# casselineau/Tracer

Hardware: AMD Instinct MI355X
Metric: Mray-bounces/s on Sandia NSTTF field (higher is better)
Workload: dtype f64

## Files before the change

tracer_amd/csrc/trc_device.h:

```cpp
#ifndef TRC_DEVICE_H
#define TRC_DEVICE_H

#include <hip/hip_runtime.h>
#include "trc_core.h"
#include "trc_bounds.h"
#include "trc_footprint.h"
#include "trc_forms.h"

struct FluxMapDev {
    int32_t surf, nu, nv, chart;
    int64_t edges_u, edges_v;
    int64_t bins;
    double proj[12];
};
static_assert(sizeof(FluxMapDev) == 136, "tests/shade_cases.py (SIZEOF_FLUXMAPDEV) restates this size in the sums of the LDS images");

struct DScene {
    const double *recs;
    const double *opt;
    const int32_t *sflags;
    const double *extra;
    int32_t stride, n_surf, n_extra, has_kd;
    const int32_t *kd_a, *kd_b, *kd_leaf, *kd_always;
    const double *kd_split;
// ... 321 lines not shown

#ifndef TALLY_PARTS
#define TALLY_PARTS 16
#endif

#define CN(k) ((k) << 4)
#define CN_WORDS (32 << 4)
enum StreamCounter {
    CW_Q1 = 0,
    CW_Q3 = 1,
    CW_HIT_LIST = 2,
    CW_ACT_OUT = 3,
    CW_OVERFLOW = 4,
    CW_ACT_IN = 5,
    CW_HITS = 6,
    CW_ALIVE = 7,
    CW_SLOTS = 8,
    CW_GEN_LIST = 9,
    CW_FP_LIST = 10,
    CW_TERM_LIST = 11,
    CW_TERM_HITS = 12,
    CW_CLS_HITS = 13,
    CW_STATS = 16,
    CW_CLS_LIST = 24
};
enum StreamOverflow : unsigned long long {
    CW_OVF_RETRY = 1,
    CW_OVF_FAIL = 2
};

struct StreamWs {
    long long cap;
    long long room;
    long long q3_cap;
    long long act_room;
    SRayGeo *geo;
    SRayAux *aux;
    uint32_t *q1_slot;
    float4 *q1_a, *q1_b;
    uint32_t *q3_slot, *q3_surf;
    SCand *q3n;
    uint32_t *hit_slot;
    uint32_t *hit_surf;
    double *hit_t;
    uint32_t *gen_list;
    uint32_t *fq_ray, *fq_cell;
    uint32_t *act[2];
// ... 32 lines not shown
    FpDev fp;
    int static_first;
    int lds_recs;
    int lds_tables;
    int lds_fm_bins;
    int lds_extra;
    int bounce_no;
    int bg_occ_words;
    int split_terminal;
    unsigned chunk_thit;
    int search;
    int shade_cls;
    int shade_term_cls;
    long long act_base0;
    unsigned chunk_hitbuf;
    const uint32_t *hl_slot, *hl_surf;
    const double *hl_t;
    long long hl_room;
    int hl_cn;
    unsigned part_chunk[3];
    int part_static[3];
    CarryIn carry;
    const float *clear_tab;
};

template <class ARGS>
__device__ __forceinline__ const ARGS *kernel_args_again() {
    static_assert(std::is_trivially_copyable<ARGS>::value, "the block is read as the bytes the launch copied into the segment");
    auto p = __builtin_amdgcn_kernarg_segment_ptr();
    asm volatile("" : "+s"(p));
    return (const ARGS *)p;
}

#define TRC_SURF_CLS_SHIFT 17
#define TRC_SURF_CLS_MASK 0x3
template <int THREADS>
__device__ __forceinline__ int wg_next(int i) {
    if constexpr (THREADS > 0) return i + THREADS;
    else return i + blockDim.x;
}

__device__ __forceinline__ void nearest_linked(const SCand *q3n, uint32_t k, double &t, int &s) {
    while (k != SQ_INVALID) {
        const SCand c = q3n[k];
        if (c.t < t || (c.t == t && (int)c.surf < s)) { t = c.t; s = (int)c.surf; }
        k = c.next;
// ... 255 lines not shown
```

tracer_amd/csrc/trc_forms.h:

```cpp
#ifndef TRC_FORMS_H
#define TRC_FORMS_H

#include <cstdio>
#include "trc_bounds.h"
#include "trc_footprint.h"

#define SC_THREADS 512
#define SC_GEN_CAP 1024
#define SF_THREADS(FLAT) ((FLAT) ? 1024 : 768)
#define SF2_DERIVES_CELL(FLAT, LDS) ((FLAT) || (LDS))
#ifndef SW_LEAFCAP
#define SW_LEAFCAP 16
#endif
#ifndef SW_LIST_T
#define SW_LIST_T uint16_t
#endif
#ifndef SW_THREADS
#define SW_THREADS 256
#endif
#define SB_THREADS 1024
#define SB_THREADS_OF(GRIDM) (SB_THREADS)
#define SA_THREADS 1024
#ifndef SHC_THREADS
#define SHC_THREADS 1024
// ... 77 lines not shown
    p.flags = flags;
    if (grid_cells) { p.grid_cells = grid_cells; p.grid_list = grid_list; }
    p.coop_waves = coop_waves;
    return p;
}
static inline size_t lds_need(const trc_lds_layout &L) { return L.end + L.slack; }
static inline size_t lds_request(const trc_lds_layout &L) { return lds_need(L) + 16; }
static inline size_t shade_lds_need(const trc_shade_parts &p) { const trc_shade_layout L = trc_shade_lds_layout(p); return L.end + L.slack; }

struct StreamKnobs {
    int search;
    bool fresh;
    bool bounce;
    bool first;
    bool coop;
    int absorb;
    bool static_chunks;
    bool room_set; long long room;
    long long q3_entries;
    int fp_cells;
    bool umask;
    int slots;
    bool clear = true;
};

struct trc_scene_facts {
    int n_surf, stride;
    bool accel_ok, accel_kd_ok, has_kd;
    int kd_nodes, kd_nleaf, kd_nalways, kd_depth;
    bool grid_ok, big_ok;
    int grid_cells, grid_list;
    int brute_list, n_unbounded;
    int big_occ_words;
    int n_fm_edges, fms_bytes, n_extra;
    long long fm_bins;
    bool chart;
    bool transfer;
    bool splits;
    bool walked;
    bool all_flat;
    bool simple;
    unsigned cls_moving, cls_all;
    bool any_term;
};
struct trc_call_facts {
    long long n;
    int flags;
    int src_kind;
    bool spec;
    bool carry;
    bool mat_dev;
    bool term_ok;
    int poly_src;
    int poly_walls;
};
struct trc_fp_facts {
    bool use;
    long long n_list;
    int M, Mc;
    bool has_generic;
    double cdf_end, coverage, ucoverage;
    int umask_words, Mu, Mv;
};
struct trc_facts { trc_scene_facts scene; trc_call_facts call; trc_fp_facts fp; StreamKnobs knobs; };

static inline void trc_scene_facts_fill(const trc_surface_desc *surfs, int n_surf, const trc_accel_host &A, bool walk, trc_scene_facts *s) {
    s->n_surf = n_surf;
    s->kd_depth = A.kd_depth;
    s->grid_ok = A.grid_ok; s->big_ok = A.big_ok;
    s->grid_cells = A.grid_off.empty() ? 0 : (int)A.grid_off.size() - 1;
    s->grid_list = (int)A.grid_list.size();
    s->brute_list = (int)A.brute_leaf.size();
    s->n_unbounded = (int)A.unbounded.size();
    s->big_occ_words = (int)A.big_occ.size();
    s->walked = walk;
    if (!walk) return;
    s->all_flat = s->simple = true;
    s->cls_moving = s->cls_all = 0u;
    s->any_term = false;
    for (int i = 0; i < n_surf; ++i) {
        const trc_surface_desc &sd = surfs[i];
        const bool flat = trc_gm_is_flat(sd.gm_kind);
        s->all_flat = s->all_flat && flat;
        s->simple = s->simple && flat && ((TRC_OPT_SIMPLE_MASK >> sd.optics_kind) & 1u);
        const unsigned bit = 1u << trc_shade_class_of(sd);
        s->cls_all |= bit;
        if (surface_ends_every_ray(sd)) s->any_term = true;
        else s->cls_moving |= bit;
    }
}

enum trc_kernel_family {
    TRC_K_NONE,
    TRC_K_CULL, TRC_K_UCULL,
    TRC_K_FRESH, TRC_K_FRESH2,
    TRC_K_BOUNCE,
    TRC_K_BOUNCE_COOP,
// ... 134 lines not shown
    return lds;
}

struct trc_stream_forms {
    int src_kind;
    int gridm;
    bool small_scene;
    trc_stage gen0, gen, walk, exact;
    trc_shade_stage shk[TRC_CLS_COUNT];
    int n_shk;
    bool multi;
    trc_stage cull, fresh, fresh_one;
    trc_stage cull_u;
    int cull_lu, cull_lv;
    double ulisted_share;
    trc_stage bounce, first, absorb;
    bool coop;
    bool use_fp, use_fused, use_first, use_absorb, absorb_inline;
    size_t lds_inline;
    double general_share;
    double listed_share;
    int search, lds_recs, lds_tally, lds_tables, lds_extra, lds_fm_bins, bg_occ_words, shade_term_cls, split_terminal;
    int poly_cells;
};

static inline trc_lds_parts trc_fresh_parts(const trc_facts &f, bool buie, bool lds, int queue_waves) {
    trc_fp_params P = {};
    P.Mc = f.fp.Mc;
    return fresh_lds_parts(f.scene.n_surf, f.scene.stride, P, f.fp.n_list, buie, lds, queue_waves);
}

static inline void trc_stream_form_general(trc_stream_forms &F, const trc_facts &f, const StreamPlan &plan) {
    const size_t b_recs = (size_t)f.scene.n_surf * f.scene.stride * 8;
    const size_t lds_exact = b_recs <= TRC_EXACT_RECS_LIMIT ? b_recs : 0;
    F.lds_recs = lds_exact ? 1 : 0;
    const int k = F.src_kind;
    const trc_kernel_id gen0 = trc_src_kind_is_lamp(k) ? trc_kid(TRC_K_GEN_LAMP, k)
                             : k == TRC_SRC_EMIT_THERMAL ? trc_kid(TRC_K_GEN_EMIT)
                             : (k == TRC_SRC_BUIE_DISK || k == TRC_SRC_PILLBOX_DISK || k == TRC_SRC_PILLBOX_RECT) ? trc_kid(TRC_K_GEN_SRC, k)
                             : trc_kid(TRC_K_GEN, 1, (k == TRC_SRC_BUIE_RECT || trc_src_kind_is_sunshape(k)) ? k : -1);
    F.gen0 = {gen0, 256, 0};
    F.gen = {trc_kid(TRC_K_GEN, 0, -1), 256, 0};
    F.walk = {trc_kid(TRC_K_WALK, SW_THREADS, plan.mode == 2), SW_THREADS, plan.lds_walk};
    F.exact = {trc_kid(TRC_K_EXACT), 256, lds_exact};
}

// ... 97 lines not shown
    F.bounce = {coop ? trc_kid(TRC_K_BOUNCE_COOP, 0, all_flat, 0) : trc_kid(TRC_K_BOUNCE, gridm, in_lds, 0, all_flat, 0), SB_THREADS_OF(gridm), request(false)};
    F.first = {coop ? trc_kid(TRC_K_BOUNCE_COOP, 1, all_flat, sun) : trc_kid(TRC_K_BOUNCE, gridm, in_lds, 1, 0, sun), SB_THREADS_OF(gridm), request(true)};
}

static inline void trc_stream_form_absorb(trc_stream_forms &F, const trc_facts &f) {
    const trc_scene_facts &sc = f.scene;
    if (!(F.use_fused && F.lds_tally && F.lds_tables && !f.call.carry)) return;
    auto need = [&](int img) { return shade_lds_need(trc_shade_lds_parts(img, true, sc.n_surf, sc.stride, sc.n_fm_edges, sc.fms_bytes, sc.n_extra, F.lds_fm_bins)); };
    const size_t lds_absorb = need(TRC_IMG_ABSORB);
    const bool fm_ok = sc.fm_bins == 0 || F.lds_fm_bins > 0;
    F.use_absorb = sc.any_term && fm_ok && !sc.chart && lds_absorb <= trc_shade_lds_limit(TRC_IMG_ABSORB, true) && !sc.transfer && f.call.term_ok && f.knobs.absorb != 0;
    if (!F.use_absorb) return;
    F.absorb = {trc_kid(TRC_K_ABSORB), SA_THREADS, lds_absorb};
    F.split_terminal = 1;
    const size_t extra_lds = need(TRC_IMG_INLINE);
    if (f.knobs.absorb != 1 && !(F.gridm == 2 && F.coop) && F.bounce.lds + extra_lds <= trc_shade_lds_limit(TRC_IMG_INLINE, true)) {
        F.absorb_inline = true;
        F.lds_inline = extra_lds;
        F.bounce.lds += extra_lds;
        F.split_terminal = 2;
    }
}

static inline bool trc_stream_decide(const trc_facts &f, const StreamPlan &plan, trc_stream_forms *out) {
    trc_stream_forms &F = *out;
    memset(&F, 0, sizeof(F));
    const int S = f.scene.n_surf;
    F.src_kind = f.call.src_kind;
    F.gridm = plan.mode == 2 ? 1 : (plan.mode == 3 ? 2 : 0);
    F.small_scene = S <= STREAM_SMALL_SURFACES && plan.mode != 1 && plan.walk_ok;
    if (F.small_scene && S <= STREAM_TINY_SURFACES) F.gridm = 3;
    F.search = plan.walk_ok ? plan.mode : 2;
    trc_stream_form_general(F, f, plan);
    if (!trc_stream_form_shade(F, f)) return false;
    trc_stream_form_fresh(F, f);
    trc_stream_form_bounce(F, f, plan);
    trc_stream_form_absorb(F, f);
    return true;
}

struct MegaPlan {
    bool m32;
    int threads;
    size_t lds;
    int lds_tally, lds_scene;
    trc_kernel_id id;
};
static inline MegaPlan mega_plan(const trc_scene_facts &sc, const trc_call_facts &c) {
    const int S = sc.n_surf;
    const bool accel = sc.has_kd && (c.flags & TRC_TRACE_ACCEL);
    const size_t b_buie = c.src_kind >= 0 ? (size_t)TRC_BUIE_STAGED * 8 : 0;
    const size_t b_tally = (size_t)(3 * S + 2) * 8;
    MegaPlan M = {false, 256, 0, 0, 0, {}};
    if (sc.accel_ok && S <= TRC_MAX_SURFACES16 && (!accel || (sc.accel_kd_ok && sc.kd_nodes <= COOP_MAX_NODES && sc.kd_depth <= COOP_MAX_DEPTH))) {
        const size_t b_acc = (size_t)6 * S * 4 + (accel ? ((size_t)2 * sc.kd_nodes * 4 + (size_t)sc.kd_nalways * 4 + (size_t)sc.kd_nleaf * 2)
                                                        : (8 + (size_t)sc.brute_list * 2)) +
                             (size_t)sc.n_unbounded * 4 + 32;
        const size_t b_wave = COOP_WAVE_BYTES(accel ? (sc.kd_depth > 0 ? sc.kd_depth : 1) : 1);
        for (int threads = 512; threads >= 256 && !M.m32; threads /= 2) {
            const size_t lds = b_buie + b_tally + b_acc + (size_t)(threads / 64) * b_wave;
// ... 42 lines not shown
```

tracer_amd/csrc/trc_shade.hip:

```cpp
#include "trc_device.h"

template <int CLS, bool FLATN, bool LDS, bool SPEC = false, bool CHART = false>
__global__ __launch_bounds__(SHC_THREADS) void k_s_shade_c(StreamParams S) {
    extern __shared__ double lds[];
    const FastParams &P = S.P;
    const DScene &sc = P.sc;
    const StreamWs &W = S.W;
    const int Sn = sc.n_surf;
    if (W.cnt[CN(CW_OVERFLOW)]) return;
    constexpr unsigned KINDS = CLS == TRC_CLS_MIRROR ? TRC_CLS_MIRROR_KINDS : TRC_CLS_DIFFUSE_KINDS;
    DScene L = sc;
    L.tally = W.tally_part + (size_t)(blockIdx.x % TALLY_PARTS) * (size_t)W.tally_n;
    double *l_tally = lds;
    double *cur = lds + (LDS ? 3 * Sn + 2 : 2);
    for (int i = threadIdx.x; i < (LDS ? 3 * Sn + 2 : 2); i += blockDim.x) l_tally[i] = 0.0;
    if (LDS) {
        double *l_recs = cur; cur += Sn * sc.stride;
        for (int i = threadIdx.x; i < Sn * sc.stride; i += blockDim.x) l_recs[i] = sc.recs[i];
        double *l_opt = cur; cur += 8 * Sn;
        for (int i = threadIdx.x; i < 8 * Sn; i += blockDim.x) l_opt[i] = sc.opt[i];
        double *l_edges = cur; cur += sc.n_fm_edges;
        for (int i = threadIdx.x; i < sc.n_fm_edges; i += blockDim.x) l_edges[i] = sc.fm_edges[i];
        FluxMapDev *l_fms = (FluxMapDev *)cur; cur += (sc.n_fm * sizeof(FluxMapDev) + 7) / 8;
        for (int i = threadIdx.x; i < sc.n_fm; i += blockDim.x) l_fms[i] = sc.fms[i];
// ... 3 lines not shown
        L.recs = l_recs; L.opt = l_opt; L.fm_edges = l_edges; L.fms = l_fms; L.fm_of_surf = l_fm_of; L.sflags = l_flags;
        cur = (double *)(((uintptr_t)(l_flags + Sn) + 7) & ~(uintptr_t)7);
        if (CLS != TRC_CLS_MIRROR) {
            double *l_extra = cur; cur += sc.n_extra;
            for (int i = threadIdx.x; i < sc.n_extra; i += blockDim.x) l_extra[i] = sc.extra[i];
            L.extra = l_extra;
        }
    }
    double *l_fm = nullptr;
    if (S.lds_fm_bins > 0) {
        l_fm = cur; cur += S.lds_fm_bins;
        for (int i = threadIdx.x; i < S.lds_fm_bins; i += blockDim.x) l_fm[i] = 0.0;
    }
    const double src_energy = P.src ? P.src->energy : 0.0;
    __syncthreads();
    long long nh = (long long)W.cnt[S.hl_cn];
    if (nh > S.hl_room) nh = S.hl_room;
    const long long padded = (nh + 63) & ~63ll;
    const unsigned wave_g = (blockIdx.x * blockDim.x + threadIdx.x) >> 6;
    WaveChunk ca = S.static_first ? chunk_init_static_at(S.chunk_act, (unsigned long long)S.act_base0 + (unsigned long long)wave_g * S.chunk_act) : chunk_init(S.chunk_act);
    WaveChunk hc = chunk_init(S.chunk_hitbuf);
    if (P.capture && wave_g < SHADE_MAX_WAVES) hit_chunk_resume(hc, W.hit_state + 2 * wave_g, S.hit_epoch);
    unsigned n_hit = 0, n_alive = 0;
    const int bounce0 = S.bounce_no;
    const bool aux_in = !P.src || bounce0 > 0;
    const long long stride = (long long)gridDim.x * blockDim.x;
    for (long long i = (long long)blockIdx.x * blockDim.x + threadIdx.x; i < padded; i += stride) {
        uint32_t slot = SQ_INVALID, hs = SQ_INVALID;
        double t = TRC_INF;
        SRayGeo g;
        g.px = g.py = g.pz = g.dx = g.dy = 0.0; g.dz = 1.0; g.head = SQ_INVALID; g.idx = 0u; g.tail = 0ull;
        bool have = false;
        if (i < nh) { slot = S.hl_slot[i]; hs = S.hl_surf[i]; t = S.hl_t[i]; }
        bool mine = false;
        int s = 0, fl = 0;
        if (slot != SQ_INVALID) {
            if (hs == SQ_INVALID) {
                g = W.geo[slot];
                have = true;
                t = TRC_INF;
                s = 0x7FFFFFFF;
                nearest_linked(W.q3n, g.head, t, s);
            } else s = (int)hs;
            if ((unsigned)s < (unsigned)Sn) {
                fl = L.sflags[s];
                const int cls = (fl >> TRC_SURF_CLS_SHIFT) & TRC_SURF_CLS_MASK;
                mine = (S.shade_term_cls >= 0 && (fl & TRC_SURF_TERMINAL)) ? (S.shade_term_cls == CLS) : (cls == CLS);
            }
            if (mine && !have) g = W.geo[slot];
        }
        const unsigned long long my_lanes = __ballot(mine);
        if (!my_lanes) continue;
        bool alive = false;
        int ts = -1;
        double tea = 0.0, tei = 0.0;
// ... 14 lines not shown
                }
                trc_normal(rec, hx, hy, hz, g.dx, g.dy, g.dz, &nx, &ny, &nz);
                trc_ray_out out[2];
                const unsigned long long rid = P.rid ? P.rid[S.base + (long long)g.idx] : (P.ray_offset + (unsigned long long)(S.base + (long long)g.idx));
                trc_shade_k<KINDS, false>(trc_rec_opt_kind(rec), L.opt + (size_t)s * 8, L.extra, trc_rec_extra_off(rec), trc_rec_extra_len(rec),
                                          rec[2], rec[5], rec[8], g.dx, g.dy, g.dz, e, 1.0, wl, 0.0, nx, ny, nz, P.seed, rid, (uint32_t)(bounce0 + 1), out);
                ox = out[0].dx; oy = out[0].dy; oz = out[0].dz; e_out = out[0].e;
            }
            const double e_abs = e - e_out;
            record_hit<LDS, CHART>(L, l_tally, s, e, e_abs, hx, hy, hz, g.dx, g.dy, g.dz, P.capture != 0, prev, &hc, l_fm, false, true);
            ts = s; tea = e_abs; tei = e;
            if (e_out > P.min_energy) {
                if (bounce0 + 1 >= P.reps) {
                    atomicAdd(&sc.counters[3], 1ull);
                    atomicAdd(sc.energy_left, e_out);
                    if (P.flags & TRC_TRACE_KEEP_LAST) {
                        const unsigned long long q = atomicAdd(&sc.counters[2], 1ull);
                        if ((long long)q < P.last_cap) {
                            P.lx[q] = hx; P.ly[q] = hy; P.lz[q] = hz;
                            P.ldx[q] = ox; P.ldy[q] = oy; P.ldz[q] = oz; P.le[q] = e_out;
                        }
                    }
                } else {
                    alive = true;
                    SRayGeo go;
                    go.px = hx; go.py = hy; go.pz = hz; go.dx = ox; go.dy = oy; go.dz = oz;
                    go.head = SQ_INVALID;
                    go.idx = g.idx;
                    uint32_t pw = (uint32_t)s;
                    if (leaves_flat(rec, hx, hy, hz, ox, oy, oz)) pw |= SQ_SKIP_SELF;
                    go.tail = sray_tail(bounce0 + 1, pw);
                    W.geo[slot] = go;
                    if (aux_in) W.aux[slot].e = e_out;
                    else { SRayAux ao; ao.e = e_out; ao.ref = SPEC ? ref0 : 1.0; ao.wl = SPEC ? wl : 0.0; ao.pad = 0.0; W.aux[slot] = ao; }
                }
            }
        }
        {
            double *tl = LDS ? l_tally : L.tally;
            unsigned long long todo = (!LDS || Sn <= 64) ? __ballot(ts >= 0) : 0ull;
            for (int round = 0; round < 6 && todo; ++round) {
                const int s0 = __shfl(ts, __ffsll((long long)todo) - 1, 64);
                const bool in = ts == s0;
                const unsigned long long m = __ballot(in);
                if (__popcll(m) < 8) break;
                const double a = wave_sum(in ? tea : 0.0), b = wave_sum(in ? tei : 0.0);
                if (lane_id() == 0) { atomicAdd(&tl[s0], a); atomicAdd(&tl[Sn + s0], b); atomicAdd(&tl[2 * Sn + s0], (double)__popcll(m)); }
                if (in) ts = -1;
                todo &= ~m;
            }
            if (ts >= 0) { atomicAdd(&tl[ts], tea); atomicAdd(&tl[Sn + ts], tei); atomicAdd(&tl[2 * Sn + ts], 1.0); }
        }
        if (P.capture) chunk_rebroadcast(hc, __ffsll((long long)my_lanes) - 1);
        const unsigned long long q = chunk_append(&W.cnt[CN(CW_ACT_OUT)], ca, alive, S.act_out, W.act_room);
        if (alive) { if ((long long)q < W.act_room) S.act_out[q] = slot; else W.cnt[CN(CW_OVERFLOW)] = CW_OVF_FAIL; n_alive += 1; }
    }
    chunk_close(ca, S.act_out, W.act_room);
    if (P.capture && wave_g < SHADE_MAX_WAVES && lane_id() == 0) hit_chunk_suspend(hc, W.hit_state + 2 * wave_g, S.hit_epoch);
    flush_counts<true>(l_tally + (LDS ? 3 * Sn : 0), n_hit, n_alive, &W.cnt[CN(CW_HITS)], &W.cnt[CN(CW_CLS_HITS + CLS)], &W.cnt[CN(CW_ALIVE)]);
    flush_sums(L.tally, l_tally, LDS ? 3 * Sn : 0, l_fm, S.lds_fm_bins, Sn);
}

template <bool LDS, bool CHART, bool SPLIT, bool MAT, bool POLY>
__device__ __forceinline__ void shade_x_body(const StreamParams &S) {
    extern __shared__ double lds[];
    const FastParams &P = S.P;
    const DScene &sc = P.sc;
    const StreamWs &W = S.W;
    const int Sn = sc.n_surf;
    if (W.cnt[CN(CW_OVERFLOW)]) return;
    DScene L = sc;
    L.tally = W.tally_part + (size_t)(blockIdx.x % TALLY_PARTS) * (size_t)W.tally_n;
    double *l_tally = lds;
    double *cur = lds + (LDS ? 3 * Sn + 2 : 2);
    for (int i = threadIdx.x; i < (LDS ? 3 * Sn + 2 : 2); i += blockDim.x) l_tally[i] = 0.0;
    if (LDS) {
        double *l_recs = cur; cur += Sn * sc.stride;
        for (int i = threadIdx.x; i < Sn * sc.stride; i += blockDim.x) l_recs[i] = sc.recs[i];
        double *l_opt = cur; cur += 8 * Sn;
        for (int i = threadIdx.x; i < 8 * Sn; i += blockDim.x) l_opt[i] = sc.opt[i];
        double *l_edges = cur; cur += sc.n_fm_edges;
        for (int i = threadIdx.x; i < sc.n_fm_edges; i += blockDim.x) l_edges[i] = sc.fm_edges[i];
// ... 338 lines not shown
```

tracer_amd/csrc/trc_stream.inc:

```


template <bool FRESH, int KIND>
__device__ __forceinline__ void s_gen_body(const StreamParams &S, trc_buie_fast &l_bf) {
    const FastParams &P = S.P;
    const DScene &sc = P.sc;
    const StreamWs &W = S.W;
    const bool buie_src = FRESH && P.src && (P.src->kind == TRC_SRC_BUIE_DISK || P.src->kind == TRC_SRC_BUIE_RECT);
    if (buie_src) trc_buie_fast_fill(P.src->buie, &l_bf, 0, (int)threadIdx.x, (int)blockDim.x);
    __syncthreads();
    if (buie_src) trc_buie_fast_fill(P.src->buie, &l_bf, 1, (int)threadIdx.x, (int)blockDim.x);
    __syncthreads();
    const trc_accel_view A = stream_accel_global(sc, S.search);
    const uint32_t *list = FRESH ? S.gen_list : S.act_in;
    long long count = FRESH ? (list ? (long long)W.cnt[CN(CW_GEN_LIST)] : S.nb) : (long long)W.cnt[CN(CW_ACT_IN)];
    if (list && count > (FRESH ? SQ_ROOM(W) : W.act_room)) count = FRESH ? SQ_ROOM(W) : W.act_room;
    const long long padded = (count + 63) & ~63ll;
    const unsigned long long wave_g = ((unsigned long long)blockIdx.x * blockDim.x + threadIdx.x) >> 6;
    WaveChunk c1 = S.static_general ? chunk_init_static(S.chunk_q1, wave_g) : chunk_init(S.chunk_q1);
    WaveChunk c3 = (!FRESH && S.q3_gen_chunk0 >= 0) ? chunk_init_static(S.chunk_q3, (unsigned long long)S.q3_gen_chunk0 + wave_g) : chunk_init(S.chunk_q3);
    WaveChunk cs = (FRESH && S.static_general) ? chunk_init_static_at(SQ_CHUNK, (unsigned long long)S.slot_base0 + wave_g * SQ_CHUNK) : chunk_init();
    for (long long i = (long long)blockIdx.x * blockDim.x + threadIdx.x; i < padded; i += (long long)gridDim.x * blockDim.x) {
        bool valid = i < count;
        uint32_t slot = 0, ri = 0;
        double px = 0, py = 0, pz = 0, dx = 0, dy = 0, dz = 1, e = 0, ref = 1.0, wl = 0.0;
// ... 1685 lines not shown
        return TRC_OK;
    }
};

#define STREAM_MAX_SLOTS 4
static StreamKnobs stream_knobs() {
    StreamKnobs K;
    const char *ev;
    K.search = (ev = getenv("TRC_STREAM_SEARCH")) ? atoi(ev) : 2;
    K.fresh = !((ev = getenv("TRC_STREAM_FRESH")) && !atoi(ev));
    K.bounce = !((ev = getenv("TRC_STREAM_BOUNCE")) && !atoi(ev));
    K.first = (ev = getenv("TRC_STREAM_FIRST")) && atoi(ev);
    K.coop = !((ev = getenv("TRC_STREAM_COOP")) && !atoi(ev));
    K.absorb = (ev = getenv("TRC_STREAM_ABSORB")) ? atoi(ev) : -1;
    K.static_chunks = !((ev = getenv("TRC_STREAM_STATIC")) && !atoi(ev));
    K.room_set = (ev = getenv("TRC_STREAM_ROOM")) != nullptr;
    K.room = K.room_set && atoll(ev) >= 64 ? atoll(ev) : 0;
    K.q3_entries = (ev = getenv("TRC_STREAM_Q3_ENTRIES")) && atoll(ev) > 0 ? atoll(ev) : 0;
    K.fp_cells = (ev = getenv("TRC_STREAM_FP_CELLS")) && atoi(ev) >= 32 ? atoi(ev) : 0;
    K.umask = !((ev = getenv("TRC_STREAM_UMASK")) && !atoi(ev));
    K.slots = (ev = getenv("TRC_STREAM_SLOTS")) ? atoi(ev) : 2;
    if (K.slots < 1 || K.slots > STREAM_MAX_SLOTS) K.slots = 2;
    K.clear = !((ev = getenv("TRC_STREAM_CLEAR")) && !atoi(ev));
    return K;
}

#define STREAM_ACT_STATIC(cap) ((cap) + ((cap) >> 2) + (1ll << 23))

static int stream_ws_alloc_queues(StreamBuffers &W, long long cap, long long want_q3, long long want_room, const StreamKnobs &K) {
    const size_t cq = (size_t)want_room;
    const long long act_room = K.room ? want_room
                             : 2 * STREAM_ACT_STATIC(cap) + cap + (1ll << 20);
    TRC_TRY(W.geo.alloc(cq));
    TRC_TRY(W.aux.alloc(cq));
    TRC_TRY(W.q1_slot.alloc(cq));
    TRC_TRY(W.q1_a.alloc(cq));
    TRC_TRY(W.q1_b.alloc(cq));
    TRC_TRY(W.q3_slot.alloc((size_t)want_q3));
    TRC_TRY(W.q3_surf.alloc((size_t)want_q3));
    TRC_TRY(W.q3n.alloc((size_t)want_q3));
    TRC_TRY(W.hit_slot.alloc(cq));
    TRC_TRY(W.hit_surf.alloc(cq));
    TRC_TRY(W.hit_t.alloc(cq));
    TRC_TRY(W.gen_list.alloc(cq));
    TRC_TRY(W.fq_ray.alloc(cq));
    TRC_TRY(W.fq_cell.alloc(cq));
// ... 46 lines not shown
    long long act_base_sh[TRC_CLS_COUNT] = {};
    unsigned gb_part = 0;
    unsigned long long part_start[TRC_CLS_COUNT] = {};
    unsigned cull_chunk = 0;
    unsigned cull_gen_chunk = 0;
    bool fresh_one = false;
    bool umask = false;
    bool fresh = false, general = false, fused = false, first = false;
    unsigned gb_first = 0;
    bool busy = false;
};

struct StreamEngine {
    StreamSlot slot[STREAM_MAX_SLOTS];
    bool ready = false;
    std::unique_ptr<trc_fp_host> fp;
    unsigned char fp_key[sizeof(int32_t) + (3 + 9 + 9 + 8) * sizeof(double)] = {};
    uint64_t fp_geom_version = 0;
    bool fp_valid = false;
    double fp_hit_rate = 0.0;
#define STREAM_RATE_BOUNCES 8
    double rate_term[STREAM_RATE_BOUNCES], rate_other[STREAM_RATE_BOUNCES];
    double rate_cls[STREAM_RATE_BOUNCES][TRC_CLS_COUNT];
    uint64_t rate_geom_version = 0;
    DevBuf<uint32_t> d_fp_mask, d_fp_coff, d_fp_umask;
    DevBuf<uint32_t> d_fp_clist;

    void forget_rates() {
        for (int b = 0; b < STREAM_RATE_BOUNCES; ++b) { rate_term[b] = rate_other[b] = -1.0; for (int c = 0; c < TRC_CLS_COUNT; ++c) rate_cls[b][c] = -1.0; }
    }
};

static void stream_fp_key(const trc_source_desc &src, unsigned char *key) {
    memcpy(key, &src.kind, sizeof(int32_t)); key += sizeof(int32_t);
    memcpy(key, src.center, 3 * sizeof(double)); key += 3 * sizeof(double);
    memcpy(key, src.rot_pos, 9 * sizeof(double)); key += 9 * sizeof(double);
    memcpy(key, src.rot_dir, 9 * sizeof(double)); key += 9 * sizeof(double);
    memcpy(key, src.p, 8 * sizeof(double));
}

static int stream_fp_prepare(trc_scene *sc, StreamEngine &E, const trc_source_desc *src, const StreamKnobs &K, FpDev *out, bool *use) {
    *use = false;
    if (!K.fresh || !src) return TRC_OK;
    unsigned char key[sizeof(E.fp_key)];
    stream_fp_key(*src, key);
    const bool buie = src->kind == TRC_SRC_BUIE_DISK || src->kind == TRC_SRC_BUIE_RECT;
    const double cdf_end = buie ? src->buie[2 * (TRC_BUIE_NELEM + 1) + TRC_BUIE_NELEM] : 0.0;
    if (!E.fp) { E.fp.reset(new (std::nothrow) trc_fp_host()); if (!E.fp) return trc_fail(TRC_ERR_NOMEM, "out of host memory"); E.fp_valid = false; }
    if (!(E.fp_valid && E.fp_geom_version == sc->search.geom_version() && memcmp(key, E.fp_key, sizeof(key)) == 0 && (!buie || E.fp->P.cdf_end == cdf_end))) {
        int M = sc->n_surf > 4096 ? 1024 : 512;
        const bool forced = K.fp_cells > 0;
        const bool um = buie;
// ... 156 lines not shown
        return trc_fail(TRC_ERR_UNSUPPORTED, "the library holds no kernel %s", name);
    }
    if (cap) TRC_TRY(kernel_grid_cap(k.fn, k.threads, lds_cap, 2048 / k.threads, n_cu, &k.max_blocks));
    return (cap && lds_cap == k.lds) ? TRC_OK : kernel_allow_lds(k.fn, k.lds);
}

static int stream_choose_forms(StreamForms &F, StreamParams &SP0, trc_scene *sc, StreamEngine &E, const StreamPlan &plan, trc_facts &f,
                               const trc_source_desc *src_desc) {
    const int n_cu = sc->ctx->n_cu;
    memset(&F, 0, sizeof(F));
    f.scene = scene_facts(sc, true);
    f.fp = {};
    TRC_TRY(stream_fp_prepare(sc, E, src_desc, f.knobs, &SP0.fp, &f.fp.use));
    if (f.fp.use) {
        const trc_fp_host &H = *E.fp;
        f.fp = {true, SP0.fp.n_list, H.P.M, H.P.Mc, H.P.has_generic != 0, H.P.cdf_end, H.coverage, H.ucoverage, E.d_fp_umask.get() ? (int)H.umask.size() : 0, H.Mu, H.Mv};
    }
    trc_stream_forms &D = F.D;
    if (!trc_stream_decide(f, plan, &D)) return trc_fail(TRC_ERR_UNSUPPORTED, "no shading kernel for device material tables beside a chart flux map");
    SP0.search = D.search; SP0.lds_recs = D.lds_recs; SP0.P.lds_tally = D.lds_tally; SP0.lds_tables = D.lds_tables; SP0.lds_extra = D.lds_extra;
    SP0.lds_fm_bins = D.lds_fm_bins; SP0.bg_occ_words = D.bg_occ_words; SP0.shade_term_cls = D.shade_term_cls; SP0.split_terminal = D.split_terminal;
    SP0.carry.poly_cells = D.poly_cells;
    SP0.clear_tab = f.knobs.clear ? sc->search.clear_cones() : nullptr;
    SP0.hit_epoch = sc->hits.epoch;
    SP0.chunk_hitbuf = sc->hits.chunk_size();
    TRC_TRY(stream_stage(F.gen0, D.gen0, n_cu, false, 0));
    TRC_TRY(stream_stage(F.gen, D.gen, n_cu, false, 0));
    TRC_TRY(stream_stage(F.walk, D.walk, n_cu, true, D.walk.lds));
    TRC_TRY(stream_stage(F.exact, D.exact, n_cu, false, 0));
    F.g_wide = (unsigned)(n_cu * 8);
    F.g_gen = (unsigned)(n_cu * 8);
    for (int q = 0; q < D.n_shk; ++q) {
        const trc_shade_stage &s = D.shk[q];
        StreamKernel k;
        const bool cap = s.id.family != TRC_K_SHADE;
        TRC_TRY(stream_stage(k, {s.id, s.threads, s.lds}, n_cu, cap, s.lds));
        StreamShadeK &K = F.shk[q];
        K = {s.cls, k.fn, (unsigned)s.threads, (unsigned)s.threads / 64, cap ? k.max_blocks : (unsigned)(n_cu * 4), s.lds, s.lds_tables, s.lds_fm_bins};
        if (cap && (unsigned long long)K.max_blocks * K.wpb > SHADE_MAX_WAVES) K.max_blocks = SHADE_MAX_WAVES / K.wpb;
    }
    TRC_TRY(stream_stage(F.cull, D.cull, n_cu, true, D.cull.lds));
    TRC_TRY(stream_stage(F.fresh, D.fresh, n_cu, true, D.fresh.lds));
    if (trc_kid_equal(D.fresh_one.id, D.fresh.id)) F.fresh_one = {F.fresh.fn, F.fresh.threads, F.fresh.lds, 0u};
    else TRC_TRY(stream_stage(F.fresh_one, D.fresh_one, n_cu, false, 0));
    TRC_TRY(stream_stage(F.cull_u, D.cull_u, n_cu, true, D.cull_u.lds));
    if (F.cull_u.fn) {
// ... 124 lines not shown
                const int c = F.shk[k].cls;
                if (!(C.K.static_chunks && T.b < STREAM_RATE_BOUNCES && E.rate_cls[T.b][c] >= 0.0)) continue;
                double cc = 1.1 * E.rate_cls[T.b][c] * rays_in0 / (double)pw + 128.0;
                const double most = (double)T.W.room / (double)pw - 64.0;
                if (cc > most) cc = most;
                unsigned chunk = ((unsigned)cc + 63u) & ~63u;
                if (chunk < SQ_CHUNK) chunk = SQ_CHUNK;
                T.SP.part_chunk[c] = chunk;
                T.SP.part_static[c] = 1;
                T.part_start[c] = pw * (unsigned long long)chunk;
                if ((long long)T.part_start[c] < entries_of[c]) entries_of[c] = (long long)T.part_start[c];
            }
        }
        unsigned long long total_waves = 0;
        for (int k = 0; k < F.D.n_shk; ++k) {
            const long long per = (long long)F.shk[k].threads * SW_ITEMS;
            const long long shade_entries_k = F.D.multi ? entries_of[F.shk[k].cls] : shade_entries;
            T.gb_sh[k] = clamp_grid((shade_entries_k + per - 1) / per, F.shk[k].max_blocks);
            total_waves += (unsigned long long)T.gb_sh[k] * F.shk[k].wpb;
        }
        const double most = (double)(C.K.room_set ? (long long)(0.9 * (double)T.W.act_room) : STREAM_ACT_STATIC(T.W.cap) - 64 * (long long)total_waves) /
                            (double)(total_waves ? total_waves : 1ull);
        const double rays_in = T.b == 0 ? (double)T.nb : (double)T.n_in;
        long long base = 0;
        for (int k = 0; k < F.D.n_shk; ++k) {
            const unsigned long long waves = (unsigned long long)T.gb_sh[k] * F.shk[k].wpb;
            unsigned chunk = SQ_CHUNK;
            if (act_expected >= 0.0) {
                double ex = act_expected;
                const int c = F.shk[k].cls;
                if (c >= 0 && T.b < STREAM_RATE_BOUNCES && E.rate_cls[T.b][c] >= 0.0 && E.rate_cls[T.b][c] * rays_in < ex) ex = E.rate_cls[T.b][c] * rays_in;
                if (C.split_rays) ex *= 2.0;
                double cc = 1.1 * ex / (double)waves + 128.0;
                if (cc > most) cc = most;
                chunk = ((unsigned)cc + 63u) & ~63u;
                if (chunk < SQ_CHUNK) chunk = SQ_CHUNK;
            }
            T.chunk_act_sh[k] = chunk;
            T.act_base_sh[k] = base;
            base += (long long)waves * (long long)chunk;
        }
        T.SP.chunk_act = T.chunk_act_sh[0];
        T.chunk_slot_sh = SQ_CHUNK;
        if (C.split_rays && total_waves) {
            double cc = 1.1 * rays_in / (double)total_waves + 64.0;
            if (cc > (double)SQ_CHUNK_MAX) cc = (double)SQ_CHUNK_MAX;
            T.chunk_slot_sh = ((unsigned)cc + 63u) & ~63u;
        }
    }
    T.gb_gen = grid_for(F.g_gen, 256 * SW_ITEMS);
    T.gb_wide = grid_for(F.g_wide, 256 * SW_ITEMS);
    T.gb_walk = grid_for(F.walk.max_blocks, SW_THREADS * SW_ITEMS);
    T.SP.chunk_q1 = work >= (1ll << 22) ? SQ_CHUNK_MAX : SQ_CHUNK;
    T.SP.chunk_q3 = work >= (1ll << 22) ? 512u : SQ_CHUNK;
    T.SP.static_first = C.K.static_chunks;
    T.SP.bounce_no = T.b;
    T.SP.static_general = C.K.static_chunks && !T.fresh;
    T.SP.q3_gen_chunk0 = (T.SP.static_general && T.b > 0) ? (long long)T.gb_walk * (SW_THREADS / 64) : -1;
    T.SP.gen_list = T.fresh ? T.SP.W.gen_list : nullptr;
// ... 197 lines not shown
    if (C.split_rays) TRC_TRY(split_ensure_room(C, T));
    TRC_TRY(upload_counters(C, T));
    return launch_bounce(C, T);
}

static int advance(StreamCall &C, StreamSlot &T) {
    StreamEngine &E = C.E;
    const unsigned long long *c = T.h_cnt.get();
#ifdef SW_STATS
    if (T.fresh) fprintf(stderr, "batch %lld: footprint list %llu entries of %lld rays (%s)\n", T.base / C.cap, c[CN(CW_FP_LIST)], T.nb, T.umask ? "umask" : "Cartesian mask");
    fprintf(stderr, "batch %lld bounce %d: Q1 %llu Q3 %llu hits %llu | walkers %llu wave-iters %llu steps %llu leaf-entries %llu box-tests %llu drains %llu drain-rounds %llu\n",
            T.base / C.cap, T.b, c[CN(CW_Q1)], c[CN(CW_Q3)], c[CN(CW_HITS)], c[CN(CW_STATS)], c[CN(CW_STATS + 1)], c[CN(CW_STATS + 2)], c[CN(CW_STATS + 3)], c[CN(CW_STATS + 4)], c[CN(CW_STATS + 5)], c[CN(CW_STATS + 6)]);
#endif
    if (c[CN(CW_OVERFLOW)]) {
        if (c[CN(CW_OVERFLOW)] != CW_OVF_RETRY || T.attempt >= 6) return trc_fail(TRC_ERR_CAPACITY, "streaming queues overflow (%llu candidate pairs, capacity %lld)", c[CN(CW_Q3)], T.W.q3_cap);
        ++T.attempt;
        TRC_TRY(T.W.grow_q3());
        T.SP.W = T.W.view();
        TRC_TRY(upload_counters(C, T));
        return launch_bounce(C, T);
    }
    T.attempt = 0;
    if (C.split_rays) T.slots_used = c[CN(CW_SLOTS)];
    C.seg += (double)T.n_in;
    C.hits += (double)c[CN(CW_HITS)];
    if (T.fresh && T.nb > 0) {
        const double rate = 1.15 * (double)c[CN(CW_HITS)] / (double)T.nb + 256.0 / (double)T.nb;
        if (rate > E.fp_hit_rate || E.fp_hit_rate > 2.0 * rate) E.fp_hit_rate = rate;
    }
    if (T.fused && T.b < STREAM_RATE_BOUNCES && T.n_in > 0) {
        const double nin = (double)T.n_in, pad = 512.0 / nin;
        const double rt = 1.15 * (double)c[CN(CW_TERM_HITS)] / nin + pad, ro = 1.15 * (double)(c[CN(CW_HITS)] - c[CN(CW_TERM_HITS)]) / nin + pad;
        if (E.rate_term[T.b] < 0.0 || rt > E.rate_term[T.b] || E.rate_term[T.b] > 2.0 * rt) E.rate_term[T.b] = rt > 1.0 ? 1.0 : rt;
        if (E.rate_other[T.b] < 0.0 || ro > E.rate_other[T.b] || E.rate_other[T.b] > 2.0 * ro) E.rate_other[T.b] = ro > 1.0 ? 1.0 : ro;
    }
    if (T.b < STREAM_RATE_BOUNCES) {
        const double rin = T.b == 0 ? (double)T.nb : (double)T.n_in;
        if (rin > 0.0)
            for (int cl = 0; cl < TRC_CLS_COUNT; ++cl) {
                const double r = 1.15 * (double)c[CN(CW_CLS_HITS + cl)] / rin + 512.0 / rin;
                double &R = E.rate_cls[T.b][cl];
                if (R < 0.0 || r > R || R > 2.0 * r) R = r;
                C.cls_hits[cl] += (double)c[CN(CW_CLS_HITS + cl)];
            }
    }
    if (T.b + 1 > C.max_bounces) C.max_bounces = T.b + 1;
    if (c[CN(CW_ALIVE)] == 0 || T.b + 1 >= C.SP0.P.reps) { T.busy = false; return TRC_OK; }
    T.n_act = c[CN(CW_ACT_OUT)];
    T.n_in = (long long)c[CN(CW_ALIVE)];
    T.SP.act_in = T.SP.W.act[T.cur];
    T.cur ^= 1;
    T.b += 1;
    if (C.split_rays) TRC_TRY(split_ensure_room(C, T));
    TRC_TRY(upload_counters(C, T));
    return launch_bounce(C, T);
}

static int stream_trace(trc_scene *sc, FastParams &P, const CarryIn &carry_in, const StreamPlan &plan, trc_facts &facts, const trc_source_desc *src_desc,
                        StreamEngine &E, trc_trace_stats *stats, double *seg_out, double *hit_out) {
    trc_ctx *ctx = sc->ctx;
    const StreamKnobs &K = facts.knobs;
    const long long cap_max = 1ll << 26;
    int n_slots = (P.n >= (1ll << 23)) ? K.slots : 1;
    long long n_batches = n_slots * ((P.n + n_slots * cap_max - 1) / (n_slots * cap_max));
    long long cap = (P.n + n_batches - 1) / n_batches;
    cap = (cap + 63) & ~63ll;
    if (cap < 64) cap = 64;
    TRC_TRY(stream_engine_init(&E, ctx));
    if (E.rate_geom_version != sc->search.geom_version()) {
// ... 77 lines not shown
```

Before: 73760.

## Finish mirror-reflected rays inside shade kernel via clear-cone lookahead intersection

In the flat mirror shade kernel, each reflected ray is checked against the precomputed clear-cone table. If it is guaranteed to escape or to hit a terminal surface, the kernel resolves it directly by brute-force testing the apartment list of surfaces. The hit is recorded and tallied there, and the ray is not re-enqueued for another bounce pass. This is meant to remove a whole bounce launch and queue traffic for most heliostat-field rays. Host-side chunk sizing gains a remaining-rays rate estimate, at the cost of extra per-ray work and divergence in the shade kernel.

```diff
diff --git a/tracer_amd/csrc/trc_device.h b/tracer_amd/csrc/trc_device.h
--- a/tracer_amd/csrc/trc_device.h
+++ b/tracer_amd/csrc/trc_device.h
@@ -367,7 +367,9 @@
     CW_TERM_HITS = 12,
     CW_CLS_HITS = 13,
     CW_STATS = 16,
-    CW_CLS_LIST = 24
+    CW_AHEAD = 23,
+    CW_CLS_LIST = 24,
+    CW_AHEAD_HITS = 27
 };
 enum StreamOverflow : unsigned long long {
     CW_OVF_RETRY = 1,
@@ -446,6 +448,7 @@
     int part_static[3];
     CarryIn carry;
     const float *clear_tab;
+    int ahead;
 };
 
 template <class ARGS>
diff --git a/tracer_amd/csrc/trc_forms.h b/tracer_amd/csrc/trc_forms.h
--- a/tracer_amd/csrc/trc_forms.h
+++ b/tracer_amd/csrc/trc_forms.h
@@ -123,6 +123,7 @@
     bool umask;
     int slots;
     bool clear = true;
+    bool ahead = true;
 };
 
 struct trc_scene_facts {
@@ -143,6 +144,7 @@
     bool simple;
     unsigned cls_moving, cls_all;
     bool any_term;
+    bool clear_cones;
 };
 struct trc_call_facts {
     long long n;
@@ -174,6 +176,7 @@
     s->brute_list = (int)A.brute_leaf.size();
     s->n_unbounded = (int)A.unbounded.size();
     s->big_occ_words = (int)A.big_occ.size();
+    s->clear_cones = A.clear_cones > 0;
     s->walked = walk;
     if (!walk) return;
     s->all_flat = s->simple = true;
@@ -354,6 +357,7 @@
     double listed_share;
     int search, lds_recs, lds_tally, lds_tables, lds_extra, lds_fm_bins, bg_occ_words, shade_term_cls, split_terminal;
     int poly_cells;
+    bool ahead;
 };
 
 static inline trc_lds_parts trc_fresh_parts(const trc_facts &f, bool buie, bool lds, int queue_waves) {
@@ -497,6 +501,17 @@
     }
 }
 
+static inline bool trc_shade_finishes_ahead(const trc_kernel_id &id) {
+    return id.family == TRC_K_SHADE_C && id.a[0] == TRC_CLS_MIRROR && id.a[1] == 1 && id.a[2] == 1 && id.a[3] == 0 && id.a[4] == 0;
+}
+
+static inline void trc_stream_form_ahead(trc_stream_forms &F, const trc_facts &f) {
+    F.ahead = false;
+    if (!(F.use_fused && F.gridm == 1 && F.bounce.id.family == TRC_K_BOUNCE && F.bounce.id.a[0] == 1 && F.bounce.id.a[2] == 0)) return;
+    if (F.split_terminal != 2 || !f.scene.clear_cones || !f.knobs.clear || f.scene.n_unbounded != 0 || !f.knobs.ahead) return;
+    for (int k = 0; k < F.n_shk; ++k) F.ahead = F.ahead || trc_shade_finishes_ahead(F.shk[k].id);
+}
+
 static inline bool trc_stream_decide(const trc_facts &f, const StreamPlan &plan, trc_stream_forms *out) {
     trc_stream_forms &F = *out;
     memset(&F, 0, sizeof(F));
@@ -511,6 +526,7 @@
     trc_stream_form_fresh(F, f);
     trc_stream_form_bounce(F, f, plan);
     trc_stream_form_absorb(F, f);
+    trc_stream_form_ahead(F, f);
     return true;
 }
 
diff --git a/tracer_amd/csrc/trc_shade.hip b/tracer_amd/csrc/trc_shade.hip
--- a/tracer_amd/csrc/trc_shade.hip
+++ b/tracer_amd/csrc/trc_shade.hip
@@ -49,6 +49,8 @@
     WaveChunk hc = chunk_init(S.chunk_hitbuf);
     if (P.capture && wave_g < SHADE_MAX_WAVES) hit_chunk_resume(hc, W.hit_state + 2 * wave_g, S.hit_epoch);
     unsigned n_hit = 0, n_alive = 0;
+    constexpr bool AHEAD = CLS == TRC_CLS_MIRROR && FLATN && LDS && !SPEC && !CHART;
+    unsigned n_ahead = 0, n_ahead_hit = 0;
     const int bounce0 = S.bounce_no;
     const bool aux_in = !P.src || bounce0 > 0;
     const long long stride = (long long)gridDim.x * blockDim.x;
@@ -58,6 +60,8 @@
         SRayGeo g;
         g.px = g.py = g.pz = g.dx = g.dy = 0.0; g.dz = 1.0; g.head = SQ_INVALID; g.idx = 0u; g.tail = 0ull;
         bool have = false;
+        int as = -1;
+        double ae = 0.0;
         if (i < nh) { slot = S.hl_slot[i]; hs = S.hl_surf[i]; t = S.hl_t[i]; }
         bool mine = false;
         int s = 0, fl = 0;
@@ -118,6 +122,42 @@
                         }
                     }
                 } else {
+                    bool ahead = false;
+                    if constexpr (AHEAD) {
+                        if (S.ahead && S.clear_tab && leaves_flat(rec, hx, hy, hz, ox, oy, oz)) {
+                            trc_ray32 r;
+                            double t0 = 0.0;
+                            bool clear = trc_ray32_prepare(sc.a_slo, sc.a_shi, sc.a_cen, hx, hy, hz, ox, oy, oz, &r, &t0) && t0 == 0.0;
+                            float tmin = 1.0f, tmax = 0.0f;
+                            if (clear && trc_kd32_root(sc.a_groot, r, &tmin, &tmax)) {
+                                const int tile = trc_clear_tile(sc.a_obb + (size_t)TRC_OBB_STRIDE * s, TRC_CLEAR_T, r.ox, r.oy, r.oz);
+                                const float4 cone = ((const float4 *)S.clear_tab)[(size_t)s * (TRC_CLEAR_T * TRC_CLEAR_T) + tile];
+                                clear = trc_clear_inside(cone.x, cone.y, cone.z, cone.w, r.dx, r.dy, r.dz);
+                            }
+                            if (clear) {
+                                double tb = TRC_INF;
+                                int sb = 0x7FFFFFFF;
+                                for (int k = 0; k < sc.a_g_napart; ++k) {
+                                    const int sidx = sc.a_gapart[k];
+                                    const float *b = sc.a_sbox + 6 * (size_t)sidx;
+                                    if ((b[3] == TRC_INF && b[0] == -TRC_INF) || sidx == s) continue;
+                                    if (!(trc_box_hit32(b, r) && trc_obb_hit32(sc.a_obb + (size_t)TRC_OBB_STRIDE * sidx, r.ox, r.oy, r.oz, r.dx, r.dy, r.dz))) continue;
+                                    const double *rec2 = L.recs + (size_t)sidx * sc.stride;
+                                    const double t2 = trc_intersect_flat(trc_rec_gm_kind(rec2), rec2, sc.extra, hx, hy, hz, ox, oy, oz);
+                                    if (t2 > 0.0 && t2 < TRC_INF && (t2 < tb || (t2 == tb && sidx < sb))) { tb = t2; sb = sidx; }
+                                }
+                                if (sb == 0x7FFFFFFF) ahead = true;
+                                else if (L.sflags[sb] & TRC_SURF_TERMINAL) {
+                                    ahead = true;
+                                    as = sb; ae = e_out;
+                                    n_ahead_hit += 1;
+                                    record_hit<LDS, CHART>(L, l_tally, sb, e_out, e_out, hx + tb * ox, hy + tb * oy, hz + tb * oz, ox, oy, oz, P.capture != 0, s, &hc, l_fm, false, true);
+                                }
+                            }
+                            if (ahead) n_ahead += 1;
+                        }
+                    }
+                    if (!ahead) {
                     alive = true;
                     SRayGeo go;
                     go.px = hx; go.py = hy; go.pz = hz; go.dx = ox; go.dy = oy; go.dz = oz;
@@ -129,6 +169,7 @@
                     W.geo[slot] = go;
                     if (aux_in) W.aux[slot].e = e_out;
                     else { SRayAux ao; ao.e = e_out; ao.ref = SPEC ? ref0 : 1.0; ao.wl = SPEC ? wl : 0.0; ao.pad = 0.0; W.aux[slot] = ao; }
+                    }
                 }
             }
         }
@@ -147,13 +188,42 @@
             }
             if (ts >= 0) { atomicAdd(&tl[ts], tea); atomicAdd(&tl[Sn + ts], tei); atomicAdd(&tl[2 * Sn + ts], 1.0); }
         }
-        if (P.capture) chunk_rebroadcast(hc, __ffsll((long long)my_lanes) - 1);
+        unsigned long long hc_lanes = my_lanes;
+        if constexpr (AHEAD) { const unsigned long long al = __ballot(as >= 0); if (al) hc_lanes = al; }
+        if (P.capture) chunk_rebroadcast(hc, __ffsll((long long)hc_lanes) - 1);
+        if constexpr (AHEAD) {
+            const unsigned long long tl = __ballot(as >= 0);
+            if (tl) {
+                const int s0 = __shfl(as, __ffsll((long long)tl) - 1, 64);
+                const bool in = as == s0;
+                const double cnt = (double)__popcll(__ballot(in));
+                const double es = wave_sum(in ? ae : 0.0);
+                if (lane_id() == 0) { atomicAdd(&l_tally[s0], es); atomicAdd(&l_tally[Sn + s0], es); atomicAdd(&l_tally[2 * Sn + s0], cnt); }
+                if (as >= 0 && !in) { atomicAdd(&l_tally[as], ae); atomicAdd(&l_tally[Sn + as], ae); atomicAdd(&l_tally[2 * Sn + as], 1.0); }
+            }
+        }
         const unsigned long long q = chunk_append(&W.cnt[CN(CW_ACT_OUT)], ca, alive, S.act_out, W.act_room);
         if (alive) { if ((long long)q < W.act_room) S.act_out[q] = slot; else W.cnt[CN(CW_OVERFLOW)] = CW_OVF_FAIL; n_alive += 1; }
     }
     chunk_close(ca, S.act_out, W.act_room);
     if (P.capture && wave_g < SHADE_MAX_WAVES && lane_id() == 0) hit_chunk_suspend(hc, W.hit_state + 2 * wave_g, S.hit_epoch);
     flush_counts<true>(l_tally + (LDS ? 3 * Sn : 0), n_hit, n_alive, &W.cnt[CN(CW_HITS)], &W.cnt[CN(CW_CLS_HITS + CLS)], &W.cnt[CN(CW_ALIVE)]);
+    if constexpr (AHEAD) {
+        if (S.ahead) {
+            double *spare = l_tally + 3 * Sn;
+            __syncthreads();
+            if (threadIdx.x == 0) spare[0] = spare[1] = 0.0;
+            __syncthreads();
+            const double a = wave_sum((double)n_ahead), h = wave_sum((double)n_ahead_hit);
+            if (lane_id() == 0 && a > 0.0) { atomicAdd(&spare[0], a); atomicAdd(&spare[1], h); }
+            __syncthreads();
+            if (threadIdx.x == 0 && spare[0] > 0.0) {
+                const unsigned long long hh = (unsigned long long)(spare[1] + 0.5);
+                atomicAdd(&W.cnt[CN(CW_AHEAD)], (unsigned long long)(spare[0] + 0.5));
+                if (hh) { atomicAdd(&W.cnt[CN(CW_AHEAD_HITS)], hh); atomicAdd(&W.cnt[CN(CW_HITS)], hh); atomicAdd(&W.cnt[CN(CW_TERM_HITS)], hh); }
+            }
+        }
+    }
     flush_sums(L.tally, l_tally, LDS ? 3 * Sn : 0, l_fm, S.lds_fm_bins, Sn);
 }
 
diff --git a/tracer_amd/csrc/trc_stream.inc b/tracer_amd/csrc/trc_stream.inc
--- a/tracer_amd/csrc/trc_stream.inc
+++ b/tracer_amd/csrc/trc_stream.inc
@@ -1731,6 +1731,7 @@
     K.slots = (ev = getenv("TRC_STREAM_SLOTS")) ? atoi(ev) : 2;
     if (K.slots < 1 || K.slots > STREAM_MAX_SLOTS) K.slots = 2;
     K.clear = !((ev = getenv("TRC_STREAM_CLEAR")) && !atoi(ev));
+    K.ahead = !((ev = getenv("TRC_STREAM_AHEAD")) && !atoi(ev));
     return K;
 }
 
@@ -1823,12 +1824,13 @@
 #define STREAM_RATE_BOUNCES 8
     double rate_term[STREAM_RATE_BOUNCES], rate_other[STREAM_RATE_BOUNCES];
     double rate_cls[STREAM_RATE_BOUNCES][TRC_CLS_COUNT];
+    double rate_left[STREAM_RATE_BOUNCES];
     uint64_t rate_geom_version = 0;
     DevBuf<uint32_t> d_fp_mask, d_fp_coff, d_fp_umask;
     DevBuf<uint32_t> d_fp_clist;
 
     void forget_rates() {
-        for (int b = 0; b < STREAM_RATE_BOUNCES; ++b) { rate_term[b] = rate_other[b] = -1.0; for (int c = 0; c < TRC_CLS_COUNT; ++c) rate_cls[b][c] = -1.0; }
+        for (int b = 0; b < STREAM_RATE_BOUNCES; ++b) { rate_term[b] = rate_other[b] = rate_left[b] = -1.0; for (int c = 0; c < TRC_CLS_COUNT; ++c) rate_cls[b][c] = -1.0; }
     }
 };
 
@@ -2031,6 +2033,7 @@
     SP0.lds_fm_bins = D.lds_fm_bins; SP0.bg_occ_words = D.bg_occ_words; SP0.shade_term_cls = D.shade_term_cls; SP0.split_terminal = D.split_terminal;
     SP0.carry.poly_cells = D.poly_cells;
     SP0.clear_tab = f.knobs.clear ? sc->search.clear_cones() : nullptr;
+    SP0.ahead = (D.ahead && SP0.clear_tab) ? 1 : 0;
     SP0.hit_epoch = sc->hits.epoch;
     SP0.chunk_hitbuf = sc->hits.chunk_size();
     TRC_TRY(stream_stage(F.gen0, D.gen0, n_cu, false, 0));
@@ -2201,6 +2204,7 @@
         const double most = (double)(C.K.room_set ? (long long)(0.9 * (double)T.W.act_room) : STREAM_ACT_STATIC(T.W.cap) - 64 * (long long)total_waves) /
                             (double)(total_waves ? total_waves : 1ull);
         const double rays_in = T.b == 0 ? (double)T.nb : (double)T.n_in;
+        const bool few_left = C.SP0.ahead && T.b < STREAM_RATE_BOUNCES && E.rate_left[T.b] >= 0.0;
         long long base = 0;
         for (int k = 0; k < F.D.n_shk; ++k) {
             const unsigned long long waves = (unsigned long long)T.gb_sh[k] * F.shk[k].wpb;
@@ -2209,11 +2213,12 @@
                 double ex = act_expected;
                 const int c = F.shk[k].cls;
                 if (c >= 0 && T.b < STREAM_RATE_BOUNCES && E.rate_cls[T.b][c] >= 0.0 && E.rate_cls[T.b][c] * rays_in < ex) ex = E.rate_cls[T.b][c] * rays_in;
+                if (few_left && E.rate_left[T.b] * rays_in < ex) ex = E.rate_left[T.b] * rays_in;
                 if (C.split_rays) ex *= 2.0;
-                double cc = 1.1 * ex / (double)waves + 128.0;
+                double cc = 1.1 * ex / (double)waves + (few_left ? 48.0 : 128.0);
                 if (cc > most) cc = most;
                 chunk = ((unsigned)cc + 63u) & ~63u;
-                if (chunk < SQ_CHUNK) chunk = SQ_CHUNK;
+                if (chunk < (few_left ? 64u : (unsigned)SQ_CHUNK)) chunk = few_left ? 64u : (unsigned)SQ_CHUNK;
             }
             T.chunk_act_sh[k] = chunk;
             T.act_base_sh[k] = base;
@@ -2457,15 +2462,16 @@
     }
     T.attempt = 0;
     if (C.split_rays) T.slots_used = c[CN(CW_SLOTS)];
-    C.seg += (double)T.n_in;
+    const unsigned long long n_ahead = c[CN(CW_AHEAD)], ahead_hits = c[CN(CW_AHEAD_HITS)];
+    C.seg += (double)T.n_in + (double)n_ahead;
     C.hits += (double)c[CN(CW_HITS)];
     if (T.fresh && T.nb > 0) {
-        const double rate = 1.15 * (double)c[CN(CW_HITS)] / (double)T.nb + 256.0 / (double)T.nb;
+        const double rate = 1.15 * (double)(c[CN(CW_HITS)] - ahead_hits) / (double)T.nb + 256.0 / (double)T.nb;
         if (rate > E.fp_hit_rate || E.fp_hit_rate > 2.0 * rate) E.fp_hit_rate = rate;
     }
     if (T.fused && T.b < STREAM_RATE_BOUNCES && T.n_in > 0) {
         const double nin = (double)T.n_in, pad = 512.0 / nin;
-        const double rt = 1.15 * (double)c[CN(CW_TERM_HITS)] / nin + pad, ro = 1.15 * (double)(c[CN(CW_HITS)] - c[CN(CW_TERM_HITS)]) / nin + pad;
+        const double rt = 1.15 * (double)(c[CN(CW_TERM_HITS)] - ahead_hits) / nin + pad, ro = 1.15 * (double)(c[CN(CW_HITS)] - c[CN(CW_TERM_HITS)]) / nin + pad;
         if (E.rate_term[T.b] < 0.0 || rt > E.rate_term[T.b] || E.rate_term[T.b] > 2.0 * rt) E.rate_term[T.b] = rt > 1.0 ? 1.0 : rt;
         if (E.rate_other[T.b] < 0.0 || ro > E.rate_other[T.b] || E.rate_other[T.b] > 2.0 * ro) E.rate_other[T.b] = ro > 1.0 ? 1.0 : ro;
     }
@@ -2479,7 +2485,16 @@
                 C.cls_hits[cl] += (double)c[CN(CW_CLS_HITS + cl)];
             }
     }
+    if (C.SP0.ahead && T.b < STREAM_RATE_BOUNCES) {
+        const double rin = T.b == 0 ? (double)T.nb : (double)T.n_in;
+        if (rin > 0.0) {
+            const double r = 1.15 * (double)c[CN(CW_ALIVE)] / rin + 512.0 / rin;
+            double &R = E.rate_left[T.b];
+            if (R < 0.0 || r > R || R > 2.0 * r) R = r;
+        }
+    }
     if (T.b + 1 > C.max_bounces) C.max_bounces = T.b + 1;
+    if (n_ahead && T.b + 2 > C.max_bounces) C.max_bounces = T.b + 2;
     if (c[CN(CW_ALIVE)] == 0 || T.b + 1 >= C.SP0.P.reps) { T.busy = false; return TRC_OK; }
     T.n_act = c[CN(CW_ACT_OUT)];
     T.n_in = (long long)c[CN(CW_ALIVE)];
```

New measurement: 83110 (median of 6 runs). +12.7%, better.
